# zrlhahaha/Direct12PBRRenderer

Hardware: AMD Instinct MI355X
Metric: shaded Mpixel/s at 4K G-buffer (full deferred frame: clustered shade + bloom + auto-exposure + ACES) (higher is better)
Workload: dtype f32

## Files before the change

direct12pbrrenderer_amd/_lib.py:

```python
import ctypes as C
import os

from .structs import CubeBc6h, CubeF32, GBuffer, Global, HaloPeer, ShadeTables, Texture2D, Tile, View

_HERE = os.path.dirname(os.path.abspath(__file__))
LIB_PATH = os.environ.get("PBR_HIP_LIB", os.path.join(_HERE, "libpbr_hip.so"))

_u32, _f32, _int, _vp, _sz = C.c_uint32, C.c_float, C.c_int, C.c_void_p, C.c_size_t

SIGNATURES = {
    "pbr_version": (C.c_char_p, []),
    "pbr_cube_texels": (_sz, [_u32, _u32]),
    "pbr_cube_mip_offset": (_sz, [_u32, _u32]),
    "pbr_env_padded_texels": (_sz, [_u32, _u32]),
    "pbr_env_padded_mip_offset": (_sz, [_u32, _u32]),
    "pbr_bloom_chain_texels": (_sz, [_u32, _u32]),
    "pbr_bloom_level_offset": (_sz, [_u32, _u32, _u32]),
    "pbr_ctx_create": (_int, [_int, C.POINTER(_vp)]),
    "pbr_ctx_destroy": (None, [_vp]),
    "pbr_ctx_set_stream": (_int, [_vp, _vp]),
    "pbr_ctx_use_own_stream": (_int, [_vp]),
    "pbr_ctx_get_stream": (_vp, [_vp]),
    "pbr_ctx_side_begin": (_int, [_vp]),
    "pbr_ctx_side_end": (_int, [_vp]),
# ... 5 lines not shown
    "pbr_cube_gen_mips": (_int, [_vp, _vp, _u32, _u32]),
    "pbr_prefilter_env": (_int, [_vp, C.POINTER(CubeF32), _u32, _u32, _vp]),
    "pbr_prefilter_env_mip": (_int, [_vp, C.POINTER(CubeF32), _u32, _u32, _f32, _vp]),
    "pbr_env_pad": (_int, [_vp, _vp, _u32, _u32, _vp]),
    "pbr_sh9_project": (_int, [_vp, C.POINTER(CubeF32), _vp]),
    "pbr_cluster_build": (_int, [_vp, C.POINTER(Global), _vp]),
    "pbr_cluster_cull": (_int, [_vp, C.POINTER(Global), _vp, _int, _vp]),
    "pbr_clustered": (_int, [_vp, C.POINTER(Global), _vp, _int, _vp]),
    "pbr_deferred_shade": (_int, [_vp, C.POINTER(Global), C.POINTER(Tile), C.POINTER(GBuffer),
                                  _vp, _u32, _vp, _u32, _u32, _vp, _vp, _int, _vp, _u32]),
    "pbr_deferred_shade_rects": (_int, [_vp, C.POINTER(Global), C.POINTER(Tile), C.POINTER(GBuffer),
                                        _vp, _u32, _vp, _u32, _u32, _vp, _vp, _int, _vp, _u32, _vp, _u32]),
    "pbr_deferred_shade_f32": (_int, [_vp, C.POINTER(Global), C.POINTER(Tile), C.POINTER(GBuffer),
                                      _vp, _u32, _vp, _u32, _u32, _vp, _vp, _int, _vp, _u32]),
    "pbr_lut_fold_x": (_int, [_vp, _vp, _u32, _vp]),
    "pbr_deferred_shade_folded": (_int, [_vp, C.POINTER(Global), C.POINTER(Tile), C.POINTER(GBuffer),
                                         _vp, _u32, _vp, _u32, _u32, _vp, _vp, _int, _vp, _u32]),
    "pbr_deferred_shade_rects_folded": (_int, [_vp, C.POINTER(Global), C.POINTER(Tile), C.POINTER(GBuffer),
                                               _vp, _u32, _vp, _u32, _u32, _vp, _vp, _int, _vp, _u32, _vp, _u32]),
    "pbr_shade_tables_bytes": (_sz, [_u32, _u32]),
    "pbr_clustered_tables": (_int, [_vp, C.POINTER(Global), _vp, _int, _vp, C.POINTER(ShadeTables)]),
    "pbr_shade_geometry_tables": (_int, [_vp, C.POINTER(Tile), C.POINTER(ShadeTables)]),
    "pbr_deferred_shade_tabled": (_int, [_vp, C.POINTER(Global), C.POINTER(Tile), C.POINTER(GBuffer),
                                         _vp, _u32, _vp, _u32, _u32, _vp, _vp, _int, _vp, _u32, C.POINTER(ShadeTables)]),
    "pbr_deferred_shade_rects_tabled": (_int, [_vp, C.POINTER(Global), C.POINTER(Tile), C.POINTER(GBuffer),
                                               _vp, _u32, _vp, _u32, _u32, _vp, _vp, _int, _vp, _u32, _vp, _u32, C.POINTER(ShadeTables)]),
    "pbr_skybox": (_int, [_vp, C.POINTER(Global), C.POINTER(Tile), C.POINTER(CubeF32), _vp, _u32, _vp, _u32]),
    "pbr_skybox_bc6h": (_int, [_vp, C.POINTER(Global), C.POINTER(Tile), C.POINTER(CubeBc6h), _vp, _u32, _vp, _u32]),
    "pbr_gbuffer_encode": (_int, [_vp, _vp, _vp, _vp, _u32, _u32, _u32, _vp, _vp, _vp]),
    "pbr_gbuffer_raster_scratch_bytes": (_sz, [_u32, _u32, _u32]),
    "pbr_gbuffer_raster_min_scratch_bytes": (_sz, [_u32, _u32, _u32]),
    "pbr_gbuffer_raster": (_int, [_vp, C.POINTER(Global), C.POINTER(Tile), _vp, _u32, _vp, _u32, _vp, _u32, _u32,
                                  _vp, _vp, _vp, _vp, _vp, _u32, _vp, _sz]),
    "pbr_texture2d_bytes": (_sz, [_u32, _u32, _u32, _u32]),
    "pbr_bc1_decode": (_int, [_vp, _vp, _u32, _u32, _u32, _u32, _vp]),
    "pbr_bc6h_chain_bytes": (_sz, [_u32, _u32]),
    "pbr_bc6h_decode_cube": (_int, [_vp, C.POINTER(_vp * 6), _u32, _u32, _vp]),
    "pbr_bc6h_encode_cube": (_int, [_vp, _vp, _u32, _u32, C.POINTER(_vp * 6)]),
    "pbr_bc6h_encode_cube_ex": (_int, [_vp, _vp, _u32, _u32, C.POINTER(_vp * 6), _u32]),
    "pbr_equirect_to_cube": (_int, [_vp, _vp, _u32, _u32, _vp, _u32, _u32, _u32]),
    "pbr_equirect_default_size": (_u32, [_u32]),
    "pbr_equirect_default_samples": (_u32, [_u32, _u32]),
    "pbr_texture2d_gen_mips": (_int, [_vp, _vp, _u32, _u32, _u32, _u32]),
    "pbr_bc1_encode": (_int, [_vp, _vp, _u32, _u32, _u32, _u32, _vp]),
    "pbr_gbuffer_raster_textured_scratch_bytes": (_sz, [_u32, _u32, _u32]),
    "pbr_gbuffer_raster_textured_min_scratch_bytes": (_sz, [_u32, _u32, _u32]),
    "pbr_gbuffer_raster_textured": (_int, [_vp, C.POINTER(Global), C.POINTER(Tile), _vp, _u32, _vp, _u32, _vp, _u32, _u32,
                                           _vp, _vp, _vp, _vp, _vp, _u32, _vp, _sz, _vp, C.POINTER(Texture2D), _u32]),
    "pbr_bloom_prefilter": (_int, [_vp, _vp, _u32, _u32, _u32, _vp, _f32, _f32]),
    "pbr_blur_h": (_int, [_vp, _vp, _u32, _u32, _vp, _u32, _u32]),
    "pbr_blur_v": (_int, [_vp, _vp, _u32, _u32, _vp, _u32, _u32]),
    "pbr_bloom_upsample_add": (_int, [_vp, _vp, _u32, _u32, _vp, _u32, _u32, _vp]),
    "pbr_bloom_up_level": (_int, [_vp, _vp, _vp, _u32, _u32, _vp, _u32, _u32]),
    "pbr_bloom_merge": (_int, [_vp, _vp, _u32, _vp, _u32, _u32]),
    "pbr_bloom": (_int, [_vp, _vp, _u32, _u32, _u32, _vp, _vp, _f32, _f32]),
    "pbr_bloom_prefilter_rect": (_int, [_vp, _vp, _u32, _u32, _u32, _vp, _u32, _u32, _u32, C.POINTER(_u32 * 4), _f32, _f32]),
    "pbr_bloom_prefilter_rects": (_int, [_vp, _vp, _u32, _u32, _u32, _vp, _u32, _u32, _u32, _vp, _u32, _f32, _f32]),
    "pbr_bloom_tiled": (_int, [_vp, _vp, _u32, C.POINTER(_u32 * 4), _u32, _u32, _vp, _vp, C.POINTER(_u32 * 4), _f32, _f32, _vp]),
    "pbr_bloom_histogram": (_int, [_vp, _vp, _u32, _u32, _u32, _vp, _vp, _f32, _f32, C.POINTER(_u32 * 4), _f32, _f32, _vp]),
    "pbr_lum_histogram": (_int, [_vp, _vp, _u32, _u32, _u32, _f32, _f32, _vp]),
    "pbr_lum_average": (_int, [_vp, _vp, _u32, _f32, _f32, _f32, _vp]),
    "pbr_tonemap": (_int, [_vp, _vp, _u32, _u32, _u32, _vp, _vp, _u32]),
    "pbr_average_tonemap": (_int, [_vp, _vp, _u32, _f32, _f32, _f32, _vp, _vp, _vp, _vp, _u32, _u32, _u32, _vp, _u32]),
    "pbr_clustered_views": (_int, [_vp, C.POINTER(View), _u32]),
    "pbr_deferred_shade_views": (_int, [_vp, C.POINTER(View), _u32, _u32, _u32, _vp, _u32, _vp, _u32, _u32]),
    "pbr_bloom_histogram_views": (_int, [_vp, C.POINTER(View), _u32, _u32, _u32, _f32, _f32, _f32, _f32]),
    "pbr_lum_average_views": (_int, [_vp, C.POINTER(View), _u32, _u32, _f32, _f32]),
    "pbr_tonemap_views": (_int, [_vp, C.POINTER(View), _u32, _u32, _u32]),
    "pbr_comm_unique_id": (_int, [_vp]),
    "pbr_comm_init": (_int, [_vp, _int, _int, _vp]),
    "pbr_allreduce_hist": (_int, [_vp, _vp]),
    "pbr_halo_staging_bytes": (_sz, [C.POINTER(HaloPeer), _u32]),
    "pbr_halo_exchange": (_int, [_vp, _vp, _u32, _u32, C.POINTER(HaloPeer), _u32, _vp, _sz]),
    "pbr_halo_pack": (_int, [_vp, _vp, _u32, _u32, C.POINTER(HaloPeer), _u32, _vp, _sz, _int]),
    "pbr_runtime_error": (C.c_char_p, []),
    "pbr_runtime_mismatch_dirs": (_int, [C.c_char_p, C.c_char_p]),
    "pbr_membench_read": (_int, [_vp, _vp, _sz, _vp, _u32]),
    "pbr_valubench": (_int, [_vp, _u32, _u32, _u32, _vp]),
    "pbr_ctx_set_bloom_shader_order": (_int, [_vp, _int]),
}

KNOBS_ONLY = {
    "pbr_ctx_set_cu_masks": (_int, [_vp, _vp, _vp, _u32]),
}

_lib = None


def load():
    global _lib
    if _lib is not None:
        return _lib
    if not os.path.exists(LIB_PATH):
        raise RuntimeError(
            f"{LIB_PATH} not found: build it with `make -C direct12pbrrenderer_amd/csrc` "
            "(or __graft_entry__.build()).  There is no CPU fallback for the HIP path.")
    import torch
    lib = C.CDLL(LIB_PATH)
    for name, (res, args) in SIGNATURES.items():
        fn = getattr(lib, name)
        fn.restype = res
        fn.argtypes = args
    for name, (res, args) in KNOBS_ONLY.items():
        fn = getattr(lib, name, None)
        if fn is not None:
            fn.restype = res
# ... 4 lines not shown
```

direct12pbrrenderer_amd/api.py:

```python
import ctypes as C

import numpy as np
import torch

from . import _lib
from .structs import (ShadeTables, Texture2D, BLOOM_KNEE, BLOOM_THRESHOLD, CLUSTER_DTYPE, ENV_MIPS, HISTOGRAM_BINS,
                      INV_LOG_LUMINANCE_RANGE, LIGHT_DTYPE, LOG_LUMINANCE_RANGE, MIN_LOG_LUMINANCE,
                      NUM_CLUSTERS, DRAW_DTYPE, DRAW_MAPS_DTYPE, BC6H_ENCODE_TWO_REGION, BC6H_MAX_SIZE, EQUIRECT_SRC_RGBE, TEX_BC1_BLOCKS, TEX_FORMATS, VERTEX_DTYPE, CubeBc6h, CubeF32, GBuffer, Global, HaloPeer, Tile, View, bloom_chain_texels, bc6h_chain_bytes, cube_texels, env_padded_texels, equirect_default_samples, equirect_default_size, texture2d_bytes)


class PbrError(RuntimeError):
    pass


def _ptr(t):
    if t is None:
        return None
    if isinstance(t, torch.Tensor):
        if not t.is_cuda:
            raise PbrError("expected a device tensor")
        if not t.is_contiguous():
            raise PbrError("expected a contiguous tensor")
        return C.c_void_p(t.data_ptr())
    return C.c_void_p(int(t))
# ... 370 lines not shown
        nbytes = texture2d_bytes(width, height, mip_levels, fmt | TEX_BC1_BLOCKS)
        if nbytes == 0 or fmt & TEX_BC1_BLOCKS:
            raise PbrError(f"bad texture description: {width} x {height}, {mip_levels} levels, stored format {stored_format}")
        if texels.numel() * texels.element_size() != texture2d_bytes(width, height, mip_levels, fmt):
            raise PbrError("bc1_encode: the texel tensor's size does not match the description")
        out = out if out is not None else self.empty((nbytes,), torch.uint8)
        if out.numel() * out.element_size() != nbytes:
            raise PbrError("bc1_encode: the output tensor's size does not match the description")
        self._check(self.lib.pbr_bc1_encode(self.h, _ptr(texels), int(width), int(height), int(mip_levels), fmt, _ptr(out)))
        return out, Texture2D(out.data_ptr(), int(width), int(height), int(mip_levels), fmt | TEX_BC1_BLOCKS)

    def import_texture(self, level0, fmt, mip_levels=None, bc1=False):
        fmt = int(fmt)
        if fmt not in TEX_FORMATS:
            raise PbrError(f"unknown texture format {fmt}")
        lv0 = np.ascontiguousarray(level0, dtype=np.uint8)
        want_dims = 2 if TEX_FORMATS[fmt][0] == 1 else 3
        if lv0.ndim != want_dims or (want_dims == 3 and lv0.shape[2] != 4):
            raise PbrError(f"import_texture: level 0 of format {fmt} is uint8 {'[h, w]' if want_dims == 2 else '[h, w, 4]'}, got {lv0.shape}")
        h, w = lv0.shape[:2]
        mips = min(w, h).bit_length() if mip_levels is None else int(mip_levels)
        nbytes = texture2d_bytes(w, h, mips, fmt)
        if nbytes == 0:
            raise PbrError(f"bad texture description: {w} x {h}, {mips} levels, format {fmt}")
        chain = self.empty((nbytes,), torch.uint8)
        chain[:lv0.size].copy_(torch.from_numpy(lv0.reshape(-1)))
        self.texture2d_gen_mips(chain, w, h, mips, fmt)
        if bc1:
            return self.bc1_encode(chain, w, h, mips, fmt)
        return chain, Texture2D(chain.data_ptr(), w, h, mips, fmt)

    def gbuffer_raster_textured(self, g: Global, tile: Tile, vertices, n_vertices, indices, n_indices, draws, n_draws, max_triangles,
                                A, B, Cc, depth, stencil, pitch, scratch, maps, textures, scratch_bytes=None):
        textures = list(textures)
        table = (Texture2D * max(len(textures), 1))(*textures)
        nbytes = scratch.numel() * scratch.element_size() if scratch_bytes is None else int(scratch_bytes)
        self._check(self.lib.pbr_gbuffer_raster_textured(
            self.h, C.byref(g), C.byref(tile), _ptr(vertices), int(n_vertices), _ptr(indices), int(n_indices), _ptr(draws),
            int(n_draws), int(max_triangles), _ptr(A), _ptr(B), _ptr(Cc), _ptr(depth), _ptr(stencil), int(pitch), _ptr(scratch),
            nbytes, _ptr(maps), table if textures else None, len(textures)))

    def bloom_prefilter(self, hdr, w, h, pitch, out, threshold=BLOOM_THRESHOLD, knee=BLOOM_KNEE):
        self._check(self.lib.pbr_bloom_prefilter(self.h, _ptr(hdr), w, h, pitch, _ptr(out), threshold, knee))

    def blur_h(self, src, iw, ih, out, ow, oh):
        self._check(self.lib.pbr_blur_h(self.h, _ptr(src), iw, ih, _ptr(out), ow, oh))

    def blur_v(self, src, iw, ih, out, ow, oh):
        self._check(self.lib.pbr_blur_v(self.h, _ptr(src), iw, ih, _ptr(out), ow, oh))

    def bloom_up_level(self, upper, lower, lw, lh, out, ow, oh):
        self._check(self.lib.pbr_bloom_up_level(self.h, _ptr(upper) if upper is not None else None, _ptr(lower), lw, lh, _ptr(out), ow, oh))

    def bloom_upsample_add(self, upper, uw, uh, lower, lw, lh, out):
        self._check(self.lib.pbr_bloom_upsample_add(self.h, _ptr(upper), uw, uh, _ptr(lower), lw, lh, _ptr(out)))

    def bloom_merge(self, hdr, pitch, src, w, h):
        self._check(self.lib.pbr_bloom_merge(self.h, _ptr(hdr), pitch, _ptr(src), w, h))

    def alloc_bloom_chain(self, w, h):
        return self.zeros((bloom_chain_texels(w, h), 4), torch.float16)

    def bloom(self, hdr, w, h, pitch, chain_a, chain_b, threshold=BLOOM_THRESHOLD, knee=BLOOM_KNEE):
        self._check(self.lib.pbr_bloom(self.h, _ptr(hdr), w, h, pitch, _ptr(chain_a), _ptr(chain_b), threshold, knee))

    def bloom_histogram(self, hdr, w, h, pitch, chain_a, chain_b, rect, hist, threshold=BLOOM_THRESHOLD, knee=BLOOM_KNEE,
                        min_log=MIN_LOG_LUMINANCE, inv_range=INV_LOG_LUMINANCE_RANGE):
        r = (C.c_uint32 * 4)(*[int(v) for v in rect])
        self._check(self.lib.pbr_bloom_histogram(self.h, _ptr(hdr), w, h, pitch, _ptr(chain_a), _ptr(chain_b), threshold, knee,
                                                 C.byref(r), min_log, inv_range, _ptr(hist)))

    def bloom_prefilter_rect(self, hdr, w, h, pitch, out, out_pitch, out_x, out_y, rect, threshold=BLOOM_THRESHOLD, knee=BLOOM_KNEE):
        r = (C.c_uint32 * 4)(*[int(v) for v in rect])
        self._check(self.lib.pbr_bloom_prefilter_rect(self.h, _ptr(hdr), w, h, pitch, _ptr(out), out_pitch, out_x, out_y,
                                                      C.byref(r), threshold, knee))

    def bloom_prefilter_rects(self, hdr, w, h, pitch, out, out_pitch, out_x, out_y, rects, threshold=BLOOM_THRESHOLD, knee=BLOOM_KNEE):
        arr = self._rects(rects)
        self._check(self.lib.pbr_bloom_prefilter_rects(self.h, _ptr(hdr), w, h, pitch, _ptr(out), out_pitch, out_x, out_y,
                                                       C.cast(arr, C.c_void_p), len(rects), threshold, knee))

    def bloom_tiled(self, hdr, hdr_pitch, hdr_rect, ew, eh, chain_a, chain_b, merge_rect, hist=None,
                    min_log=MIN_LOG_LUMINANCE, inv_range=INV_LOG_LUMINANCE_RANGE):
        hr = (C.c_uint32 * 4)(*[int(v) for v in hdr_rect])
        mr = (C.c_uint32 * 4)(*[int(v) for v in merge_rect])
        self._check(self.lib.pbr_bloom_tiled(self.h, _ptr(hdr), hdr_pitch, C.byref(hr), ew, eh, _ptr(chain_a), _ptr(chain_b),
                                             C.byref(mr), min_log, inv_range, _ptr(hist)))

    def lum_histogram(self, hdr, w, h, pitch, hist, min_log=MIN_LOG_LUMINANCE, inv_range=INV_LOG_LUMINANCE_RANGE):
        self._check(self.lib.pbr_lum_histogram(self.h, _ptr(hdr), w, h, pitch, min_log, inv_range, _ptr(hist)))

    def lum_average(self, hist, pixel_count, dt, avg, min_log=MIN_LOG_LUMINANCE, log_range=LOG_LUMINANCE_RANGE):
        self._check(self.lib.pbr_lum_average(self.h, _ptr(hist), pixel_count, min_log, log_range, dt, _ptr(avg)))

    def tonemap(self, hdr, w, h, pitch, avg, out, out_pitch):
        self._check(self.lib.pbr_tonemap(self.h, _ptr(hdr), w, h, pitch, _ptr(avg), _ptr(out), out_pitch))

    def average_tonemap(self, hist, pixel_count, dt, avg_in, avg_out, hist_clear, hdr, w, h, pitch, out, out_pitch,
                        min_log=MIN_LOG_LUMINANCE, log_range=LOG_LUMINANCE_RANGE):
        self._check(self.lib.pbr_average_tonemap(self.h, _ptr(hist), pixel_count, min_log, log_range, dt, _ptr(avg_in), _ptr(avg_out),
                                                 _ptr(hist_clear) if hist_clear is not None else None, _ptr(hdr), w, h, pitch, _ptr(out), out_pitch))

    def clustered_views(self, views, n):
        self._check(self.lib.pbr_clustered_views(self.h, views, n))

    def deferred_shade_views(self, views, n, w, h, lut, lut_res, env, env_size, env_mips):
# ... 59 lines not shown
```

direct12pbrrenderer_amd/csrc/bloom.hip:

```cpp
#include <type_traits>
#include "pbr_internal.hpp"
#include "pbr_device.hpp"

using namespace pbr;

__constant__ float c_gauss[9] = {0.0148f, 0.0459f, 0.1050f, 0.1941f, 0.2803f, 0.1941f, 0.1050f, 0.0459f, 0.0148f};

__device__ __forceinline__ float4 to4(F4 v) { return make_float4(v.x, v.y, v.z, v.w); }
__device__ __forceinline__ F4 from4(float4 v) { return f4(v.x, v.y, v.z, v.w); }

struct OutRect { int x0, y0, x1, y1, ox, oy, pitch; };
constexpr int PF_MAX_RECTS = 5;
struct OutRects {
    int n, ox, oy, pitch;
    int x0[PF_MAX_RECTS], y0[PF_MAX_RECTS], x1[PF_MAX_RECTS], y1[PF_MAX_RECTS], tiles_x[PF_MAX_RECTS], first[PF_MAX_RECTS + 1];
};
__device__ __forceinline__ float4 soft_knee_sample(F4 c, float threshold, float knee) {
    const float brightness = fmaxf(c.x, fmaxf(c.y, c.z));
    float soft = fminf(fmaxf(brightness - threshold + threshold * knee, 0.0f), 2.0f * threshold * knee);
    soft /= 4.0f * threshold * knee + 0.00001f;
    const float contribution = fmaxf(soft, brightness - threshold) / fmaxf(brightness, 0.00001f);
    const float cr = c.x * contribution, cg = c.y * contribution, cb = c.z * contribution;
    const float wgt = 1.0f / (luminance(cr, cg, cb) + 1.0f);
    return make_float4(cr * wgt, cg * wgt, cb * wgt, wgt);
// ... 627 lines not shown
                                lineU[0][uq] = make_float2((float)hupE.x, (float)hupO.x); lineU[1][uq] = make_float2((float)hupE.y, (float)hupO.y);
                                lineU[2][uq] = make_float2((float)hupE.z, (float)hupO.z);
                            }
                            wave_sync();
                            V3 uE, uO;
                            gauss9_pair(lineU[0] + lane, uE.x, uO.x); gauss9_pair(lineU[1] + lane, uE.y, uO.y); gauss9_pair(lineU[2] + lane, uE.z, uO.z);
                            wave_sync();
                            bE = bE + uE; bO = bO + uO;
                        }
                        struct alignas(16) H8 { H4 a, b; } th;
                        th.a.x = to_half_rn(bE.x); th.a.y = to_half_rn(bE.y); th.a.z = to_half_rn(bE.z); th.a.w = alpha.t;
                        th.b.x = to_half_rn(bO.x); th.b.y = to_half_rn(bO.y); th.b.z = to_half_rn(bO.z); th.b.w = alpha.t;
                        *reinterpret_cast<H8*>(&sT[r][2 * lane]) = th;
                    }
                }
                pE = cE; pO = cO;
            }
        }
    }
    __syncthreads();
    {
        H4 win[PER_O + 8];
#pragma unroll
        for (int i = 0; i < PER_O + 8; i++) win[i] = sT[rbase + i][vc];
#pragma unroll
        for (int k = 0; k < PER_O; k++) {
            const int y = y0 + rbase + k;
            if (xv >= ow || y >= oh) continue;
            V3 a3 = v3(0.0f, 0.0f, 0.0f);
#pragma unroll
            for (int i = 0; i < 9; i++) a3 = fma3(h3f(win[k + i]), c_gauss[i], a3);
            const F4 a = f4(a3.x, a3.y, a3.z, alpha.v);
            if (TAIL == 0) {
                store_h4(out + 4 * ((size_t)y * out_pitch + xv), a);
            } else {
                if (!(merge_has(tr, in_mx, y))) continue;
                const H4Packed o = merge_rounded_packed(a3, a0w, h4f(hdr_in[k]));
                *reinterpret_cast<H4Packed*>(hdr_row0 + k * hdr_pitch + hdr_x) = o;
                if (TAIL == 2) {
                    if (hist_has(tr, xv, y))
                        atomicAdd(&sh_hist[wv][luminance_bin_exact((float)o.lo.x, (float)o.lo.y, (float)o.hi.x, min_log, inv_range)], 1u);
                }
            }
        }
    }
    if (tile + (int)gridDim.x < n_tiles) __syncthreads();
    }
    if (TAIL == 2) {
        __syncthreads();
        hist_flush<NT>(sh_hist, t, hist);
    }
}

template <bool DUAL>
static pbr_status launch_blur_h(pbr_ctx* ctx, const pbr_half* in, uint32_t iw, uint32_t ih, const pbr_half* in2, uint32_t iw2, uint32_t ih2,
                                pbr_half* out, uint32_t ow, uint32_t oh) {
    const uint64_t row_blocks = (uint64_t)((ow + 255) / 256) * oh;
    int rows = (int)(row_blocks / 2048);
    rows = rows < 1 ? 1 : (rows > HB_MAX_ROWS ? HB_MAX_ROWS : rows);
    hipLaunchKernelGGL(k_blur_h<DUAL>, dim3((ow + 255) / 256, (oh + rows - 1) / rows), dim3(256), 0, ctx->stream, in, (int)iw, (int)ih, in2, (int)iw2, (int)ih2,
                       out, (int)ow, (int)oh, 1.0f / (float)ow, 1.0f / (float)oh, rows);
    return launched(ctx, DUAL ? "k_blur_h<dual>" : "k_blur_h");
}

static bool exact_half(uint32_t n) { return (n & 1u) == 0u && n <= 8192u; }

static TailRect tail_rect(uint32_t ow, uint32_t oh, const uint32_t* rect, const uint32_t* merge_rect, const uint32_t* buf_origin) {
    TailRect tr{};
    if (rect) { tr.hx0 = (int)rect[0]; tr.hy0 = (int)rect[1]; tr.hx1 = (int)(rect[0] + rect[2]); tr.hy1 = (int)(rect[1] + rect[3]); }
    tr.mx1 = (int)ow; tr.my1 = (int)oh;
    if (merge_rect) {
        tr.mx0 = (int)merge_rect[0]; tr.my0 = (int)merge_rect[1];
        tr.mx1 = (int)(merge_rect[0] + merge_rect[2]); tr.my1 = (int)(merge_rect[1] + merge_rect[3]);
    }
    if (buf_origin) { tr.bx = (int)buf_origin[0]; tr.by = (int)buf_origin[1]; }
    return tr;
}
struct TileGrid { int tx0, ty0, tiles_x, n; };
static TileGrid tile_grid(const TailRect& tr, int tw, int th) {
    const int tx0 = tr.mx0 / tw, ty0 = tr.my0 / th, tiles_x = (tr.mx1 + tw - 1) / tw - tx0;
    return TileGrid{tx0, ty0, tiles_x, tiles_x * ((tr.my1 + th - 1) / th - ty0)};
}

template <int MODE, bool DUAL, int TAIL, bool MV = false>
static pbr_status launch_hv(pbr_ctx* ctx, const LevelViews& lv, uint32_t nv, uint32_t iw, uint32_t ih, uint32_t ow, uint32_t oh,
                            const uint32_t* rect, float min_log, float inv_range,
                            const uint32_t* merge_rect = nullptr, const uint32_t* buf_origin = nullptr) {
    using VS = std::conditional_t<MV, LevelViews, NoViews>;
    VS vs{};
    if constexpr (MV) vs = lv;
    TailRect tr = tail_rect(ow, oh, rect, merge_rect, buf_origin);
    static const int hist_blocks = pbr::knob_int("PBR_BLOOM_HIST_BLOCKS", 1024);
    auto even_blocks = [nv](int n_tiles) { const int per = (n_tiles * (int)nv + hist_blocks - 1) / hist_blocks; return (n_tiles + per - 1) / per; };
    auto launch = [&](auto kernel, const TileGrid& g, const char* label) {
        tr.tx0 = g.tx0; tr.ty0 = g.ty0;
        hipLaunchKernelGGL(kernel, dim3(TAIL == 2 ? even_blocks(g.n) : g.n, nv), dim3(512), 0, ctx->stream,
                           MV ? nullptr : lv.in[0], (int)iw, (int)ih, MV ? nullptr : lv.in2[0], MV ? nullptr : lv.out[0], (int)ow, (int)oh,
                           MV ? 0 : lv.out_pitch[0], g.tiles_x, g.n, tr, min_log, inv_range, vs, MV ? nullptr : lv.hist[0]);
        return launched(ctx, label);
    };
    if constexpr (MODE == M_UP) {
        static const int wide_forced = pbr::knob_int("PBR_BLOOM_WIDE", -1);
        const TileGrid wide = tile_grid(tr, 128, 32);
        if (wide_forced >= 0 ? wide_forced == 1 : (wide.n >= 400 && !ctx->bloom_shader_order))
            return launch(k_blur_up_poly<DUAL, TAIL, 32, VS>, wide, MV ? "k_blur_up_poly<views>" : "k_blur_up_poly");
    }
// ... 97 lines not shown
    if (!ctx) return PBR_ERR_INVALID;
    PBR_REQUIRE(ctx, hdr && out && rects && n_rects >= 1 && n_rects <= (uint32_t)PF_MAX_RECTS, "pbr_bloom_prefilter_rects: null pointer / 1 .. 5 rectangles");
    PBR_CHECK(ctx, "pbr_bloom_prefilter_rects", prefilter_image_fault(w, h, pitch));
    PBR_REQUIRE(ctx, prefilter_dest_ok(out_pitch, out_y), "pbr_bloom_prefilter_rects: bad size");
    for (uint32_t r = 0; r < n_rects; r++)
        PBR_REQUIRE(ctx, !prefilter_rect_fault(rects[r], w, h, out_x, out_pitch), "pbr_bloom_prefilter_rects: rectangle outside the half-res image / the output pitch");
    return prefilter_rects(ctx, hdr, w, h, pitch, out, out_pitch, out_x, out_y, rects, n_rects, threshold, knee);
}

pbr_status pbr_blur_h(pbr_ctx* ctx, const pbr_half* in, uint32_t iw, uint32_t ih, pbr_half* out, uint32_t ow, uint32_t oh) {
    if (!ctx) return PBR_ERR_INVALID;
    PBR_REQUIRE(ctx, in && out, "pbr_blur_h: null pointer");
    PBR_REQUIRE(ctx, iw && ih && ow && oh && iw <= 65535 && ih <= 65535 && ow <= 65535 && oh <= 65535, "pbr_blur_h: bad size");
    return launch_blur_h<false>(ctx, in, iw, ih, nullptr, 0, 0, out, ow, oh);
}

pbr_status pbr_blur_v(pbr_ctx* ctx, const pbr_half* in, uint32_t iw, uint32_t ih, pbr_half* out, uint32_t ow, uint32_t oh) {
    if (!ctx) return PBR_ERR_INVALID;
    PBR_REQUIRE(ctx, in && out, "pbr_blur_v: null pointer");
    PBR_REQUIRE(ctx, iw && ih && ow && oh && iw <= 65535 && ih <= 65535 && ow <= 65535 && oh <= 65535, "pbr_blur_v: bad size");
    const float tx = 1.0f / (float)ow, ty = 1.0f / (float)oh;
    dim3 grid((ow + VT_W - 1) / VT_W, (oh + VT_R - 1) / VT_R);
    hipLaunchKernelGGL(k_blur_v, grid, dim3(VT_W, 4), 0, ctx->stream, in, (int)iw, (int)ih, out, (int)ow, (int)oh, tx, ty);
    return launched(ctx, "k_blur_v");
}

pbr_status pbr_bloom_upsample_add(pbr_ctx* ctx, const pbr_half* upper, uint32_t uw, uint32_t uh,
                                  const pbr_half* lower, uint32_t lw, uint32_t lh, pbr_half* out) {
    if (!ctx) return PBR_ERR_INVALID;
    PBR_REQUIRE(ctx, upper && lower && out, "pbr_bloom_upsample_add: null pointer");
    PBR_REQUIRE(ctx, uw && uh && lw && lh && uw <= 65535 && uh <= 65535, "pbr_bloom_upsample_add: bad size");
    return launch_blur_h<true>(ctx, lower, lw, lh, upper, uw, uh, out, uw, uh);
}

pbr_status pbr_bloom_merge(pbr_ctx* ctx, pbr_half* hdr, uint32_t pitch, const pbr_half* in, uint32_t w, uint32_t h) {
    if (!ctx) return PBR_ERR_INVALID;
    PBR_REQUIRE(ctx, hdr && in, "pbr_bloom_merge: null pointer");
    PBR_REQUIRE(ctx, w && h && w <= 65535 && h <= 65535 && pitch >= w, "pbr_bloom_merge: bad size");
    dim3 grid((w + 255) / 256, h);
    hipLaunchKernelGGL(k_bloom_merge, grid, dim3(256), 0, ctx->stream, hdr, (int)pitch, in, (int)w, (int)h);
    return launched(ctx, "k_bloom_merge");
}

pbr_status pbr_bloom_up_level(pbr_ctx* ctx, const pbr_half* upper, const pbr_half* lower, uint32_t lw, uint32_t lh,
                              pbr_half* out, uint32_t ow, uint32_t oh) {
    if (!ctx) return PBR_ERR_INVALID;
    PBR_REQUIRE(ctx, lower && out && out != lower && out != upper, "pbr_bloom_up_level: null pointer / out aliases an input");
    PBR_REQUIRE(ctx, lw >= 1 && lh >= 1 && ow == 2 * lw && oh == 2 * lh && exact_half(ow) && exact_half(oh), "pbr_bloom_up_level: out must be exactly twice lower, even, <= 8192");
    const LevelViews lv = level_views(1, [&](uint32_t) { return LevelIO{lower, upper, out, (int)ow, nullptr}; });
    if (upper) return launch_hv<M_UP, true, 0>(ctx, lv, 1, lw, lh, ow, oh, nullptr, 0.0f, 0.0f);
    return launch_hv<M_UP, false, 0>(ctx, lv, 1, lw, lh, ow, oh, nullptr, 0.0f, 0.0f);
}

}

static pbr_status bloom_final(pbr_ctx* ctx, const pbr_half* b0, pbr_half* hdr, uint32_t w, uint32_t h, uint32_t pitch,
                              const uint32_t* hist_rect, float min_log, float inv_range, uint32_t* hist256) {
    const float tx = 1.0f / (float)w, ty = 1.0f / (float)h;
    const int tiles_x = (int)((w + VT_W - 1) / VT_W), tiles_y = (int)((h + VT_R - 1) / VT_R);
    int blocks = tiles_x * tiles_y;
    if (blocks > 1280) blocks = 1280;
    if (hist256) {
        hipLaunchKernelGGL(k_blur_v_merge<true>, dim3(blocks), dim3(VT_W, 4), 0, ctx->stream, b0, (int)w, (int)h, tx, ty, hdr, (int)pitch, tiles_x, tiles_y,
                           (int)hist_rect[0], (int)hist_rect[1], (int)(hist_rect[0] + hist_rect[2]), (int)(hist_rect[1] + hist_rect[3]), min_log, inv_range, hist256);
    } else {
        hipLaunchKernelGGL(k_blur_v_merge<false>, dim3(blocks), dim3(VT_W, 4), 0, ctx->stream, b0, (int)w, (int)h, tx, ty, hdr, (int)pitch, tiles_x, tiles_y,
                           0, 0, 0, 0, 0.0f, 0.0f, (uint32_t*)nullptr);
    }
    return launched(ctx, "k_blur_v_merge");
}

static void up_pass_rects(const uint32_t merge0[4], uint32_t w, uint32_t h, uint32_t need[PBR_BLOOM_MIPS][4]) {
    int x0 = (int)merge0[0], y0 = (int)merge0[1], x1 = (int)(merge0[0] + merge0[2]), y1 = (int)(merge0[1] + merge0[3]);
    for (uint32_t l = 1; l < PBR_BLOOM_MIPS; l++) {
        const int lw = (int)(w >> l), lh = (int)(h >> l);
        x0 = (x0 - 4) / 2 - 2; y0 = (y0 - 4) / 2 - 2; x1 = (x1 + 4 + 1) / 2 + 2; y1 = (y1 + 4 + 1) / 2 + 2;
        x0 = x0 < 0 ? 0 : x0; y0 = y0 < 0 ? 0 : y0; x1 = x1 > lw ? lw : x1; y1 = y1 > lh ? lh : y1;
        need[l][0] = (uint32_t)x0; need[l][1] = (uint32_t)y0; need[l][2] = (uint32_t)(x1 - x0); need[l][3] = (uint32_t)(y1 - y0);
    }
}

struct BloomView { pbr_half* hdr; uint32_t pitch; pbr_half* A; pbr_half* B; uint32_t* hist; };

template <bool MV>
static pbr_status bloom_pass(pbr_ctx* ctx, const BloomView* v, uint32_t n, uint32_t w, uint32_t h, bool prefilter, float threshold, float knee,
                             const uint32_t* hist_rect, float min_log, float inv_range, const uint32_t* merge0 = nullptr, const uint32_t* origin = nullptr) {
    auto W = [&](uint32_t l) { return w >> l; };
    auto H = [&](uint32_t l) { return h >> l; };
    auto off = [&](uint32_t l) { return (size_t)4 * pbr_bloom_level_offset(w, h, l); };
    auto exact = [&](uint32_t l) { return exact_half(W(l)) && exact_half(H(l)); };
    pbr_status r;
    if (prefilter) {
        const OutRect whole{0, 0, (int)W(1), (int)H(1), 0, 0, (int)W(1)};
        if (MV && exact(0)) {
            PrefilterViews pv{};
            for (uint32_t i = 0; i < n; i++) { pv.hdr[i] = v[i].hdr; pv.out[i] = v[i].A + off(1); pv.pitch[i] = (int)v[i].pitch; }
            const OutRects rs = out_rects(&whole, 1);
            hipLaunchKernelGGL(k_bloom_prefilter_2x<PrefilterViews>, dim3(rs.first[1], n), dim3(256), 0, ctx->stream,
                               nullptr, (int)w, (int)h, 0, pv, nullptr, rs, threshold, knee);
            if ((r = launched(ctx, "k_bloom_prefilter_2x<views>"))) return r;
        } else {
            for (uint32_t i = 0; i < n; i++)
                if ((r = prefilter_launch(ctx, v[i].hdr, w, h, v[i].pitch, v[i].A + off(1), &whole, 1, threshold, knee))) return r;
        }
    }
    for (uint32_t k = 0; k < PBR_BLOOM_STEP; k++) {
        const uint32_t up = k + 1, lo = k + 2;
        if (exact(up)) {
            const LevelViews lv = level_views(n, [&](uint32_t i) { return LevelIO{v[i].A + off(up), nullptr, v[i].A + off(lo), (int)W(lo), nullptr}; });
            if ((r = launch_hv<M_DOWN, false, 0, MV>(ctx, lv, n, W(up), H(up), W(lo), H(lo), nullptr, 0.0f, 0.0f))) return r;
        } else {
            for (uint32_t i = 0; i < n; i++) {
                if ((r = pbr_blur_h(ctx, v[i].A + off(up), W(up), H(up), v[i].B + off(lo), W(lo), H(lo)))) return r;
                if ((r = pbr_blur_v(ctx, v[i].B + off(lo), W(lo), H(lo), v[i].A + off(lo), W(lo), H(lo)))) return r;
            }
        }
    }
    uint32_t need[PBR_BLOOM_MIPS][4];
    static const bool shrink = pbr::knob_int("PBR_BLOOM_SHRINK", 1) != 0;
    const bool use_need = merge0 != nullptr && shrink;
    if (use_need) up_pass_rects(merge0, w, h, need);
    bool res_in_b = false;
    uint32_t res_level = PBR_BLOOM_MIPS - 1;
    auto res = [&](uint32_t i) { return (const pbr_half*)(res_in_b ? v[i].B : v[i].A) + off(res_level); };
    for (int k = PBR_BLOOM_STEP - 1; k >= 0; k--) {
        const uint32_t up = (uint32_t)k + 1;
        if (exact(up)) {
            const LevelViews lv = level_views(n, [&](uint32_t i) { return LevelIO{res(i), v[i].A + off(up), v[i].B + off(up), (int)W(up), nullptr}; });
            if ((r = launch_hv<M_UP, true, 0, MV>(ctx, lv, n, W(up + 1), H(up + 1), W(up), H(up), nullptr, 0.0f, 0.0f,
                                                  use_need ? need[up] : nullptr))) return r;
            res_in_b = true;
        } else {
            for (uint32_t i = 0; i < n; i++) {
                if ((r = pbr_bloom_upsample_add(ctx, v[i].A + off(up), W(up), H(up), res(i), W(up + 1), H(up + 1), v[i].B + off(up)))) return r;
                if ((r = pbr_blur_v(ctx, v[i].B + off(up), W(up), H(up), v[i].A + off(up), W(up), H(up)))) return r;
            }
            res_in_b = false;
        }
        res_level = up;
    }
    if (exact(0)) {
        const LevelViews lv = level_views(n, [&](uint32_t i) { return LevelIO{res(i), nullptr, v[i].hdr, (int)v[i].pitch, v[i].hist}; });
        if constexpr (!MV)
            if (!v[0].hist) return launch_hv<M_UP, false, 1>(ctx, lv, 1, w >> 1, h >> 1, w, h, nullptr, 0.0f, 0.0f, merge0, origin);
        return launch_hv<M_UP, false, 2, MV>(ctx, lv, n, w >> 1, h >> 1, w, h, hist_rect, min_log, inv_range, merge0, origin);
    }
    for (uint32_t i = 0; i < n; i++) {
        if ((r = pbr_blur_h(ctx, res(i), w >> 1, h >> 1, v[i].B, w, h))) return r;
        if ((r = bloom_final(ctx, v[i].B, v[i].hdr, w, h, v[i].pitch, hist_rect, min_log, inv_range, v[i].hist))) return r;
    }
    return PBR_OK;
}

extern "C" {

static pbr_status bloom_impl(pbr_ctx* ctx, pbr_half* hdr, uint32_t w, uint32_t h, uint32_t pitch, pbr_half* A, pbr_half* B,
                             float threshold, float knee, const uint32_t* hist_rect, float min_log, float inv_range, uint32_t* hist256) {
    PBR_REQUIRE(ctx, hdr && A && B, "pbr_bloom: null pointer");
    PBR_CHECK(ctx, "pbr_bloom", chain_size_fault(w, h, pitch));
    const BloomView v{hdr, pitch, A, B, hist256};
    return bloom_pass<false>(ctx, &v, 1, w, h, true, threshold, knee, hist_rect, min_log, inv_range);
}

pbr_status pbr_bloom(pbr_ctx* ctx, pbr_half* hdr, uint32_t w, uint32_t h, uint32_t pitch,
                     pbr_half* A, pbr_half* B, float threshold, float knee) {
    if (!ctx) return PBR_ERR_INVALID;
    return bloom_impl(ctx, hdr, w, h, pitch, A, B, threshold, knee, nullptr, 0.0f, 0.0f, nullptr);
}

pbr_status pbr_bloom_histogram(pbr_ctx* ctx, pbr_half* hdr, uint32_t w, uint32_t h, uint32_t pitch,
                               pbr_half* A, pbr_half* B, float threshold, float knee,
                               const uint32_t rect[4], float min_log, float inv_range, uint32_t* hist256) {
    if (!ctx) return PBR_ERR_INVALID;
    PBR_REQUIRE(ctx, rect && hist256, "pbr_bloom_histogram: null pointer");
    PBR_REQUIRE(ctx, rect[2] >= 1 && rect[3] >= 1 && rect[0] + rect[2] <= w && rect[1] + rect[3] <= h, "pbr_bloom_histogram: rect outside the image");
    return bloom_impl(ctx, hdr, w, h, pitch, A, B, threshold, knee, rect, min_log, inv_range, hist256);
}

pbr_status pbr_bloom_histogram_views(pbr_ctx* ctx, const pbr_view* views, uint32_t n, uint32_t w, uint32_t h,
// ... 42 lines not shown
```

include/pbr_hip.h:

```cpp
#ifndef PBR_HIP_H
#define PBR_HIP_H

#include <stdint.h>
#include <stddef.h>

#ifdef __cplusplus
extern "C" {
#endif

typedef int pbr_status;
enum {
    PBR_OK              =  0,
    PBR_ERR_INVALID     = -1,
    PBR_ERR_HIP         = -2,
    PBR_ERR_NOMEM       = -3,
    PBR_ERR_UNSUPPORTED = -4,
    PBR_ERR_COMM        = -5
};

typedef struct pbr_ctx pbr_ctx;
typedef uint16_t pbr_half;

#define PBR_CLUSTER_X              24
#define PBR_CLUSTER_Y              16
// ... 224 lines not shown
#define PBR_RASTER_MAX_SIZE      8192u
size_t pbr_gbuffer_raster_scratch_bytes(uint32_t w, uint32_t h, uint32_t n_triangles);
size_t pbr_gbuffer_raster_min_scratch_bytes(uint32_t w, uint32_t h, uint32_t n_triangles);
pbr_status pbr_gbuffer_raster(pbr_ctx* ctx, const pbr_global* g, const pbr_tile* tile,
                              const pbr_vertex* vertices, uint32_t n_vertices, const uint32_t* indices, uint32_t n_indices,
                              const pbr_draw* draws, uint32_t n_draws, uint32_t max_triangles,
                              uint32_t* A, uint32_t* B, uint32_t* C, float* depth, uint8_t* stencil, uint32_t pitch,
                              void* scratch, size_t scratch_bytes);

#define PBR_TEX_R8G8B8A8_UNORM       28u
#define PBR_TEX_B8G8R8A8_UNORM       87u
#define PBR_TEX_B8G8R8A8_UNORM_SRGB  91u
#define PBR_TEX_R8_UNORM             61u
#define PBR_TEX_MAX_SIZE             16384u
#define PBR_TEX_BC1_BLOCKS           0x100u
typedef struct pbr_texture2d {
    const void* texels;
    uint32_t width, height;
    uint32_t mip_levels;
    uint32_t format;
} pbr_texture2d;
size_t pbr_texture2d_bytes(uint32_t width, uint32_t height, uint32_t mip_levels, uint32_t format);
pbr_status pbr_bc1_decode(pbr_ctx* ctx, const void* blocks, uint32_t width, uint32_t height, uint32_t mip_levels,
                          uint32_t stored_format, void* out);
pbr_status pbr_texture2d_gen_mips(pbr_ctx* ctx, void* texels, uint32_t width, uint32_t height, uint32_t mip_levels, uint32_t format);
pbr_status pbr_bc1_encode(pbr_ctx* ctx, const void* texels, uint32_t width, uint32_t height, uint32_t mip_levels,
                          uint32_t stored_format, void* blocks_out);
#define PBR_NO_MAP                   0xffffffffu
#define PBR_RASTER_MAX_TEXTURES      64u
typedef struct pbr_draw_maps {
    uint32_t albedo, normal, roughness, metallic, ao;
} pbr_draw_maps;
size_t pbr_gbuffer_raster_textured_scratch_bytes(uint32_t w, uint32_t h, uint32_t n_triangles);
size_t pbr_gbuffer_raster_textured_min_scratch_bytes(uint32_t w, uint32_t h, uint32_t n_triangles);
pbr_status pbr_gbuffer_raster_textured(pbr_ctx* ctx, const pbr_global* g, const pbr_tile* tile,
                                       const pbr_vertex* vertices, uint32_t n_vertices, const uint32_t* indices, uint32_t n_indices,
                                       const pbr_draw* draws, uint32_t n_draws, uint32_t max_triangles,
                                       uint32_t* A, uint32_t* B, uint32_t* C, float* depth, uint8_t* stencil, uint32_t pitch,
                                       void* scratch, size_t scratch_bytes,
                                       const pbr_draw_maps* maps, const pbr_texture2d* textures, uint32_t n_textures);

pbr_status pbr_bloom_prefilter(pbr_ctx* ctx, const pbr_half* hdr, uint32_t w, uint32_t h,
                               uint32_t pitch, pbr_half* out, float threshold, float knee);
pbr_status pbr_blur_h(pbr_ctx* ctx, const pbr_half* in, uint32_t iw, uint32_t ih,
                      pbr_half* out, uint32_t ow, uint32_t oh);
pbr_status pbr_blur_v(pbr_ctx* ctx, const pbr_half* in, uint32_t iw, uint32_t ih,
                      pbr_half* out, uint32_t ow, uint32_t oh);
pbr_status pbr_bloom_upsample_add(pbr_ctx* ctx, const pbr_half* upper, uint32_t uw, uint32_t uh,
                                  const pbr_half* lower, uint32_t lw, uint32_t lh, pbr_half* out);
pbr_status pbr_bloom_merge(pbr_ctx* ctx, pbr_half* hdr, uint32_t pitch, const pbr_half* in,
                           uint32_t w, uint32_t h);
pbr_status pbr_bloom_up_level(pbr_ctx* ctx, const pbr_half* upper, const pbr_half* lower, uint32_t lw, uint32_t lh,
                              pbr_half* out, uint32_t ow, uint32_t oh);
pbr_status pbr_bloom(pbr_ctx* ctx, pbr_half* hdr, uint32_t w, uint32_t h, uint32_t pitch,
                     pbr_half* chain_a, pbr_half* chain_b, float threshold, float knee);

pbr_status pbr_bloom_prefilter_rect(pbr_ctx* ctx, const pbr_half* hdr, uint32_t w, uint32_t h, uint32_t pitch,
                                    pbr_half* out, uint32_t out_pitch, uint32_t out_x, uint32_t out_y,
                                    const uint32_t rect[4], float threshold, float knee);
pbr_status pbr_bloom_prefilter_rects(pbr_ctx* ctx, const pbr_half* hdr, uint32_t w, uint32_t h, uint32_t pitch,
                                     pbr_half* out, uint32_t out_pitch, uint32_t out_x, uint32_t out_y,
                                     const uint32_t (*rects)[4], uint32_t n_rects, float threshold, float knee);
pbr_status pbr_bloom_tiled(pbr_ctx* ctx, pbr_half* hdr, uint32_t hdr_pitch, const uint32_t hdr_rect[4],
                           uint32_t ew, uint32_t eh, pbr_half* chain_a, pbr_half* chain_b, const uint32_t merge_rect[4],
                           float min_log, float inv_range, uint32_t* hist256);

pbr_status pbr_bloom_histogram(pbr_ctx* ctx, pbr_half* hdr, uint32_t w, uint32_t h, uint32_t pitch,
                               pbr_half* chain_a, pbr_half* chain_b, float threshold, float knee,
                               const uint32_t rect[4], float min_log, float inv_range, uint32_t* hist256);

pbr_status pbr_lum_histogram(pbr_ctx* ctx, const pbr_half* hdr, uint32_t w, uint32_t h,
                             uint32_t pitch, float min_log, float inv_range, uint32_t* hist256);
pbr_status pbr_lum_average(pbr_ctx* ctx, uint32_t* hist256, uint32_t pixel_count, float min_log,
                           float range, float delta_time, float* avg_inout);
pbr_status pbr_tonemap(pbr_ctx* ctx, const pbr_half* hdr, uint32_t w, uint32_t h, uint32_t pitch,
                       const float* avg, uint32_t* rgba8, uint32_t out_pitch);
pbr_status pbr_average_tonemap(pbr_ctx* ctx, const uint32_t* hist256, uint32_t pixel_count, float min_log, float range, float delta_time,
                               const float* avg_in, float* avg_out, uint32_t* hist_clear256,
                               const pbr_half* hdr, uint32_t w, uint32_t h, uint32_t pitch, uint32_t* rgba8, uint32_t out_pitch);

#define PBR_MAX_VIEWS 16
typedef struct pbr_view {
    pbr_global       g;
    pbr_gbuffer      gb;
    const pbr_light* lights;
    int32_t          num_lights;
    pbr_cluster*     clusters;
    pbr_half*        hdr;
    uint32_t         hdr_pitch;
    pbr_half*        chain_a;
    pbr_half*        chain_b;
    uint32_t*        hist256;
    float*           avg;
    uint32_t*        rgba8;
    uint32_t         out_pitch;
} pbr_view;

pbr_status pbr_clustered_views(pbr_ctx* ctx, const pbr_view* views, uint32_t n);
pbr_status pbr_deferred_shade_views(pbr_ctx* ctx, const pbr_view* views, uint32_t n, uint32_t w, uint32_t h,
                                    const pbr_half* lut, uint32_t lut_res,
                                    const pbr_half* env_padded, uint32_t env_size, uint32_t env_mips);
pbr_status pbr_bloom_histogram_views(pbr_ctx* ctx, const pbr_view* views, uint32_t n, uint32_t w, uint32_t h,
                                     float threshold, float knee, float min_log, float inv_range);
pbr_status pbr_lum_average_views(pbr_ctx* ctx, const pbr_view* views, uint32_t n, uint32_t pixel_count, float min_log, float range);
pbr_status pbr_tonemap_views(pbr_ctx* ctx, const pbr_view* views, uint32_t n, uint32_t w, uint32_t h);

// ... 27 lines not shown
```

Measured before the change: 18980.

## Fuse bloom levels 3-4 down and up passes into one LDS-resident kernel

Adds a kernel that computes the downsample to level 3, its blur, the downsample to level 4, its blur, and the upsample-add back to level 3 for one output tile, keeping every intermediate in LDS. It replaces two down-step launches and one up-step launch in the single-view bloom path, removing those launches and the global-memory round trips for the small mips. In exchange, each tile recomputes a halo cone of level-3 and level-4 texels, and the large LDS footprint per block may limit occupancy. The new path can be turned off with an environment knob.

```diff
diff --git a/direct12pbrrenderer_amd/_lib.py b/direct12pbrrenderer_amd/_lib.py
--- a/direct12pbrrenderer_amd/_lib.py
+++ b/direct12pbrrenderer_amd/_lib.py
@@ -81,6 +81,7 @@
     "pbr_blur_v": (_int, [_vp, _vp, _u32, _u32, _vp, _u32, _u32]),
     "pbr_bloom_upsample_add": (_int, [_vp, _vp, _u32, _u32, _vp, _u32, _u32, _vp]),
     "pbr_bloom_up_level": (_int, [_vp, _vp, _vp, _u32, _u32, _vp, _u32, _u32]),
+    "pbr_bloom_levels34": (_int, [_vp, _vp, _u32, _u32, _vp]),
     "pbr_bloom_merge": (_int, [_vp, _vp, _u32, _vp, _u32, _u32]),
     "pbr_bloom": (_int, [_vp, _vp, _u32, _u32, _u32, _vp, _vp, _f32, _f32]),
     "pbr_bloom_prefilter_rect": (_int, [_vp, _vp, _u32, _u32, _u32, _vp, _u32, _u32, _u32, C.POINTER(_u32 * 4), _f32, _f32]),
diff --git a/direct12pbrrenderer_amd/api.py b/direct12pbrrenderer_amd/api.py
--- a/direct12pbrrenderer_amd/api.py
+++ b/direct12pbrrenderer_amd/api.py
@@ -446,6 +446,9 @@
     def bloom_up_level(self, upper, lower, lw, lh, out, ow, oh):
         self._check(self.lib.pbr_bloom_up_level(self.h, _ptr(upper) if upper is not None else None, _ptr(lower), lw, lh, _ptr(out), ow, oh))
 
+    def bloom_levels34(self, a2, w2, h2, b3):
+        self._check(self.lib.pbr_bloom_levels34(self.h, _ptr(a2), w2, h2, _ptr(b3)))
+
     def bloom_upsample_add(self, upper, uw, uh, lower, lw, lh, out):
         self._check(self.lib.pbr_bloom_upsample_add(self.h, _ptr(upper), uw, uh, _ptr(lower), lw, lh, _ptr(out)))
 
diff --git a/direct12pbrrenderer_amd/csrc/bloom.hip b/direct12pbrrenderer_amd/csrc/bloom.hip
--- a/direct12pbrrenderer_amd/csrc/bloom.hip
+++ b/direct12pbrrenderer_amd/csrc/bloom.hip
@@ -703,6 +703,145 @@
     }
 }
 
+struct L34 {
+    static constexpr int NT = 512, TW = 32, TH = 16;
+    static constexpr int UW = TW + 8, UH = TH + 8;
+    static constexpr int C4W = TW / 2 + 6, C4H = TH / 2 + 6;
+    static constexpr int S4W = C4W + 8, H4H = C4H + 8;
+    static constexpr int A3W = 2 * S4W, A3H = 2 * H4H;
+    static constexpr int S3W = A3W + 8, H3H = A3H + 8;
+    static constexpr int NS = S3W * H3H, NH = A3W * H3H;
+    static_assert(S4W * H4H <= NS && 2 * UW * UH <= NS && C4W * H4H <= NH && TW * UH <= NH, "later regions reuse the first level's storage");
+    static_assert(NT >= S3W && NT >= A3W, "a thread owns one column of a region");
+};
+
+template <int NT, int SW, int OW, int ROWS, bool DUAL>
+__device__ __forceinline__ void l34_h_pass(const float4* s, const float4* s2, H4* out, h16 alpha_t, int t) {
+    for (int e = t; e < OW * ROWS; e += NT) {
+        const int j = e / OW, i = e - j * OW;
+        V3 g = gauss9_rgb(s + j * SW + i);
+        if (DUAL) g = g + gauss9_rgb(s2 + j * SW + i);
+        H4 th;
+        th.x = to_half_rn(g.x); th.y = to_half_rn(g.y); th.z = to_half_rn(g.z); th.w = alpha_t;
+        out[e] = th;
+    }
+}
+template <int NT, int OW, int OH, int HROWS, class Store>
+__device__ __forceinline__ void l34_v_pass(const H4* hreg, int ox, int oy, int hy0, int lw, int lh, int t, Store store) {
+    constexpr int G = NT / OW, R = (OH + G - 1) / G;
+    const int grp = t / OW, i = t - grp * OW, x = ox + i, j0 = grp * R;
+    if (grp >= G || j0 >= OH || x < 0 || x >= lw) return;
+    H4 win[R + 8];
+#pragma unroll
+    for (int m = 0; m < R + 8; m++) win[m] = hreg[clampi(clampi(oy + j0 - 4 + m, 0, lh - 1) - hy0, 0, HROWS - 1) * OW + i];
+#pragma unroll
+    for (int k = 0; k < R; k++) {
+        const int j = j0 + k, y = oy + j;
+        if (j >= OH || y < 0 || y >= lh) continue;
+        V3 a3 = v3(0.0f, 0.0f, 0.0f);
+#pragma unroll
+        for (int n = 0; n < 9; n++) a3 = fma3(h3f(win[k + n]), c_gauss[n], a3);
+        store(i, j, x, y, a3);
+    }
+}
+
+__global__ __launch_bounds__(L34::NT) void k_bloom_levels34(const pbr_half* __restrict__ a2, int w3, int h3, pbr_half* __restrict__ b3) {
+    using C = L34;
+    constexpr int NT = C::NT, TW = C::TW, TH = C::TH, UW = C::UW, UH = C::UH, C4W = C::C4W, C4H = C::C4H, S4W = C::S4W, H4H = C::H4H,
+                  A3W = C::A3W, A3H = C::A3H, S3W = C::S3W, H3H = C::H3H;
+    __shared__ float4 sS[C::NS];
+    __shared__ H4 sH[C::NH];
+    __shared__ H4 sA3[A3W * A3H];
+    __shared__ H4 sA4[C4W * C4H];
+    static_assert(sizeof(sS) + sizeof(sH) + sizeof(sA3) + sizeof(sA4) <= 160 * 1024, "k_bloom_levels34: the cone no longer fits the LDS");
+    const int t = threadIdx.x;
+    const int w2 = 2 * w3, w4 = w3 >> 1, h4 = h3 >> 1;
+    const int x0 = blockIdx.x * TW, y0 = blockIdx.y * TH;
+    const int ox4 = (x0 >> 1) - 3, oy4 = (y0 >> 1) - 3;
+    const int ox3 = 2 * (ox4 - 4), oy3 = 2 * (oy4 - 4);
+    const h16 a2w = reinterpret_cast<const H4*>(a2)[0].w;
+    {
+        constexpr int G = NT / S3W, K = (H3H + G - 1) / G;
+        struct alignas(16) Pair { H4 lo, hi; };
+        const int rg = t / S3W, i = t - rg * S3W, p = ox3 - 4 + i;
+        const Pair* col = reinterpret_cast<const Pair*>(a2) + (clampi(2 * p, 0, w2 - 2) >> 1);
+        Pair r0[K], r1[K];
+        if (rg < G) {
+#pragma unroll
+            for (int k = 0; k < K; k++) {
+                const int yc = clampi(oy3 - 4 + min(rg + k * G, H3H - 1), 0, h3 - 1);
+                r0[k] = col[(size_t)(2 * yc) * w3];
+                r1[k] = col[(size_t)(2 * yc + 1) * w3];
+            }
+#pragma unroll
+            for (int k = 0; k < K; k++) {
+                if (rg + k * G >= H3H) break;
+                Tap2 tap;
+                tap.c00 = p >= w3 ? r0[k].hi : r0[k].lo; tap.c10 = p < 0 ? r0[k].lo : r0[k].hi;
+                tap.c01 = p >= w3 ? r1[k].hi : r1[k].lo; tap.c11 = p < 0 ? r1[k].lo : r1[k].hi;
+                sS[(rg + k * G) * S3W + i] = finish_tap2_rgb<M_DOWN>(tap, 0.5f, 0.5f);
+            }
+        }
+    }
+    const h16 t3 = to_half_rn(gauss9_const((float)a2w));
+    const h16 a3w = to_half_rn(gauss9_const((float)t3));
+    const h16 t4 = to_half_rn(gauss9_const((float)a3w));
+    const h16 a4w = to_half_rn(gauss9_const((float)t4));
+    float alpha_h = gauss9_const((float)a4w);
+    alpha_h = alpha_h + gauss9_const((float)a3w);
+    const h16 tu = to_half_rn(alpha_h);
+    const float alpha_v = gauss9_const((float)tu);
+    __syncthreads();
+    l34_h_pass<NT, S3W, A3W, H3H, false>(sS, nullptr, sH, t3, t);
+    __syncthreads();
+    l34_v_pass<NT, A3W, A3H, H3H>(sH, ox3, oy3, oy3 - 4, w3, h3, t, [&](int i, int j, int, int, V3 a) {
+        H4 o;
+        o.x = to_half_rn(a.x); o.y = to_half_rn(a.y); o.z = to_half_rn(a.z); o.w = a3w;
+        sA3[j * A3W + i] = o;
+    });
+    __syncthreads();
+    auto a3_at = [&](int x, int y) { return sA3[clampi(y - oy3, 0, A3H - 1) * A3W + clampi(x - ox3, 0, A3W - 1)]; };
+    for (int e = t; e < S4W * H4H; e += NT) {
+        const int j = e / S4W, i = e - j * S4W;
+        int ax0, ax1, ay0, ay1;
+        float fx, fy;
+        tap1d<M_DOWN>(ox4 - 4 + i, w3, ax0, ax1, fx);
+        tap1d<M_DOWN>(clampi(oy4 - 4 + j, 0, h4 - 1), h3, ay0, ay1, fy);
+        const Tap2 tap{a3_at(ax0, ay0), a3_at(ax1, ay0), a3_at(ax0, ay1), a3_at(ax1, ay1)};
+        sS[e] = finish_tap2_rgb<M_DOWN>(tap, fx, fy);
+    }
+    __syncthreads();
+    l34_h_pass<NT, S4W, C4W, H4H, false>(sS, nullptr, sH, t4, t);
+    __syncthreads();
+    l34_v_pass<NT, C4W, C4H, H4H>(sH, ox4, oy4, oy4 - 4, w4, h4, t, [&](int i, int j, int, int, V3 a) {
+        H4 o;
+        o.x = to_half_rn(a.x); o.y = to_half_rn(a.y); o.z = to_half_rn(a.z); o.w = a4w;
+        sA4[j * C4W + i] = o;
+    });
+    __syncthreads();
+    auto a4_at = [&](int x, int y) { return sA4[clampi(y - oy4, 0, C4H - 1) * C4W + clampi(x - ox4, 0, C4W - 1)]; };
+    float4* const sU = sS;
+    float4* const sL = sS + UW * UH;
+    for (int e = t; e < UW * UH; e += NT) {
+        const int j = e / UW, i = e - j * UW;
+        const int p = x0 - 4 + i, yr = clampi(y0 - 4 + j, 0, h3 - 1);
+        int ax0, ax1, ay0, ay1;
+        float fx, fy;
+        tap1d<M_UP>(p, w4, ax0, ax1, fx);
+        tap1d<M_UP>(yr, h4, ay0, ay1, fy);
+        const Tap2 tap{a4_at(ax0, ay0), a4_at(ax1, ay0), a4_at(ax0, ay1), a4_at(ax1, ay1)};
+        sU[e] = finish_tap2_rgb<M_UP>(tap, fx, fy);
+        const H4 up = a3_at(clampi(p, 0, w3 - 1), yr);
+        sL[e] = make_float4((float)up.x, (float)up.y, (float)up.z, 0.0f);
+    }
+    __syncthreads();
+    l34_h_pass<NT, UW, TW, UH, true>(sU, sL, sH, tu, t);
+    __syncthreads();
+    l34_v_pass<NT, TW, TH, UH>(sH, x0, y0, y0 - 4, w3, h3, t, [&](int, int, int x, int y, V3 a) {
+        store_h4(b3 + 4 * ((size_t)y * w3 + x), f4(a.x, a.y, a.z, alpha_v));
+    });
+}
+
 template <bool DUAL>
 static pbr_status launch_blur_h(pbr_ctx* ctx, const pbr_half* in, uint32_t iw, uint32_t ih, const pbr_half* in2, uint32_t iw2, uint32_t ih2,
                                 pbr_half* out, uint32_t ow, uint32_t oh) {
@@ -906,6 +1045,23 @@
     return launch_hv<M_UP, false, 0>(ctx, lv, 1, lw, lh, ow, oh, nullptr, 0.0f, 0.0f);
 }
 
+static bool levels34_ok(const pbr_half* a2, uint32_t w2, uint32_t h2) {
+    return (pbr::addr(a2) & 15u) == 0 && exact_half(w2) && exact_half(h2) && exact_half(w2 >> 1) && exact_half(h2 >> 1) && (w2 >> 2) >= 1 && (h2 >> 2) >= 1;
+}
+static pbr_status launch_levels34(pbr_ctx* ctx, const pbr_half* a2, uint32_t w2, uint32_t h2, pbr_half* b3) {
+    const uint32_t w3 = w2 >> 1, h3 = h2 >> 1;
+    hipLaunchKernelGGL(k_bloom_levels34, dim3((w3 + L34::TW - 1) / L34::TW, (h3 + L34::TH - 1) / L34::TH), dim3(L34::NT), 0, ctx->stream,
+                       a2, (int)w3, (int)h3, b3);
+    return launched(ctx, "k_bloom_levels34");
+}
+
+pbr_status pbr_bloom_levels34(pbr_ctx* ctx, const pbr_half* a2, uint32_t w2, uint32_t h2, pbr_half* b3) {
+    if (!ctx) return PBR_ERR_INVALID;
+    PBR_REQUIRE(ctx, a2 && b3 && a2 != b3, "pbr_bloom_levels34: null pointer / out aliases the input");
+    PBR_REQUIRE(ctx, levels34_ok(a2, w2, h2), "pbr_bloom_levels34: level 2 must halve exactly twice (sides multiples of 4, <= 8192) and be 16-byte aligned");
+    return launch_levels34(ctx, a2, w2, h2, b3);
+}
+
 }
 
 static pbr_status bloom_final(pbr_ctx* ctx, const pbr_half* b0, pbr_half* hdr, uint32_t w, uint32_t h, uint32_t pitch,
@@ -958,8 +1114,12 @@
                 if ((r = prefilter_launch(ctx, v[i].hdr, w, h, v[i].pitch, v[i].A + off(1), &whole, 1, threshold, knee))) return r;
         }
     }
+    static_assert(PBR_BLOOM_STEP == 3 && PBR_BLOOM_MIPS == 5, "the levels-3-and-4 launch replaces down steps 1, 2 and up step 2");
+    static const bool levels34_on = pbr::knob_int("PBR_BLOOM_LEVELS34", 1) != 0;
+    const bool levels34 = !MV && n == 1 && !merge0 && !ctx->bloom_shader_order && levels34_on && exact(1) && levels34_ok(v[0].A + off(2), W(2), H(2));
     for (uint32_t k = 0; k < PBR_BLOOM_STEP; k++) {
         const uint32_t up = k + 1, lo = k + 2;
+        if (levels34 && k >= 1) break;
         if (exact(up)) {
             const LevelViews lv = level_views(n, [&](uint32_t i) { return LevelIO{v[i].A + off(up), nullptr, v[i].A + off(lo), (int)W(lo), nullptr}; });
             if ((r = launch_hv<M_DOWN, false, 0, MV>(ctx, lv, n, W(up), H(up), W(lo), H(lo), nullptr, 0.0f, 0.0f))) return r;
@@ -979,6 +1139,12 @@
     auto res = [&](uint32_t i) { return (const pbr_half*)(res_in_b ? v[i].B : v[i].A) + off(res_level); };
     for (int k = PBR_BLOOM_STEP - 1; k >= 0; k--) {
         const uint32_t up = (uint32_t)k + 1;
+        if (levels34 && up == 3) {
+            if ((r = launch_levels34(ctx, v[0].A + off(2), W(2), H(2), v[0].B + off(3)))) return r;
+            res_in_b = true;
+            res_level = 3;
+            continue;
+        }
         if (exact(up)) {
             const LevelViews lv = level_views(n, [&](uint32_t i) { return LevelIO{res(i), v[i].A + off(up), v[i].B + off(up), (int)W(up), nullptr}; });
             if ((r = launch_hv<M_UP, true, 0, MV>(ctx, lv, n, W(up + 1), H(up + 1), W(up), H(up), nullptr, 0.0f, 0.0f,
diff --git a/include/pbr_hip.h b/include/pbr_hip.h
--- a/include/pbr_hip.h
+++ b/include/pbr_hip.h
@@ -300,6 +300,7 @@
                            uint32_t w, uint32_t h);
 pbr_status pbr_bloom_up_level(pbr_ctx* ctx, const pbr_half* upper, const pbr_half* lower, uint32_t lw, uint32_t lh,
                               pbr_half* out, uint32_t ow, uint32_t oh);
+pbr_status pbr_bloom_levels34(pbr_ctx* ctx, const pbr_half* a2, uint32_t w2, uint32_t h2, pbr_half* b3);
 pbr_status pbr_bloom(pbr_ctx* ctx, pbr_half* hdr, uint32_t w, uint32_t h, uint32_t pitch,
                      pbr_half* chain_a, pbr_half* chain_b, float threshold, float knee);
 
```

Result: no change. 19100, median of 5 (+0.7%).
